# Parskatt/RoMa

Hardware: AMD Instinct MI355X
Metric: image-pairs/sec, roma_outdoor 560->864, batch=8 per GPU (higher is better)
Workload: dtype bf16; 1 GPU; roma_outdoor match() 560->864, symmetric, upsample_preds, 8 pairs/GPU/step, seeded synthetic weights + N(0,1) images; precision policy of the reference's bf16 timing script: bfloat16 DINOv2 + float16 autocast for VGG / decoder / refiners (ROMA_MIXED), f32 accumulate; precision_policy=mixed, global_batch=8, streams_per_gpu=2, parallelism=single GPU, outputs_finite=True

## Files before the change

### include/roma_hip.h

```cpp
#ifndef ROMA_HIP_H
#define ROMA_HIP_H
#include <stdint.h>
#ifdef __cplusplus
extern "C" {
#endif

typedef struct roma_model* roma_handle_t;

enum { ROMA_F32 = 0, ROMA_BF16 = 1, ROMA_F16 = 2,
       ROMA_MIXED = 3 };
int roma_h16_format(void);
enum { ROMA_ERR_ARG = -1, ROMA_ERR_HIP = -2, ROMA_ERR_STATE = -3 };

typedef struct {
  int coarse_h, coarse_w;
  int upsample_h, upsample_w;
  int symmetric;
  int upsample_preds;
  int attenuate_cert;
  int precision;
  int max_batch;
  int device;
} roma_config_t;

// ... 111 lines not shown
int roma_op_multinomial(const float* weights, long n, long k, unsigned long long seed, long long* out_indices, void* workspace,
                        long workspace_bytes, void* stream);
long roma_op_ransac_workspace(int B, int N);
int roma_op_ransac(int model, const float* kpts_a, const float* kpts_b, const int* counts, const unsigned long long* seeds, int B,
                   int N, float threshold, double confidence, int max_iters, int refine, double* out_model, unsigned char* out_mask,
                   unsigned char* out_ok, int* out_info, void* workspace, long workspace_bytes, void* stream);
long roma_op_magsac_workspace(int B, int N);
int roma_op_magsac(int model, const float* kpts_a, const float* kpts_b, const int* counts, const unsigned long long* seeds, int B,
                   int N, float threshold, double confidence, int max_iters, int lo_iters, double* out_model, unsigned char* out_mask,
                   unsigned char* out_ok, int* out_info, double* out_score, void* workspace, long workspace_bytes, void* stream);
long roma_op_essential_workspace(int B, int N);
int roma_op_essential(const float* kpts_a, const float* kpts_b, const int* counts, const unsigned long long* seeds,
                      const double* camera_matrix, int B, int N, float threshold, double prob, int max_iters, double* out_e,
                      unsigned char* out_mask, unsigned char* out_ok, int* out_info, void* workspace, long workspace_bytes,
                      void* stream);
long roma_op_essential_magsac_workspace(int B, int N);
int roma_op_essential_magsac(const float* kpts_a, const float* kpts_b, const int* counts, const unsigned long long* seeds,
                             const double* camera_matrix, int B, int N, float threshold, double prob, int max_iters, int lo_iters,
                             double* out_e, unsigned char* out_mask, unsigned char* out_ok, int* out_info, double* out_score,
                             void* workspace, long workspace_bytes, void* stream);
int roma_op_essential_minimal(const double* x0, const double* x1, int S, double* out_e, int* out_n, void* stream);
long roma_op_recover_pose_workspace(int B, int N);
int roma_op_recover_pose(const double* E, const float* kpts_a, const float* kpts_b, const unsigned char* mask, const int* counts,
                         const double* camera_matrix, int B, int N, double distance_thresh, int* out_n_good, double* out_r,
                         double* out_t, unsigned char* out_mask, void* workspace, long workspace_bytes, void* stream);
long roma_op_refine_pose_workspace(int B, int N);
int roma_op_refine_pose(const double* R, const double* t, const float* kpts_a, const float* kpts_b, const int* counts,
                        const unsigned char* valid, int B, int N, double thr, int max_steps, double* out_r, double* out_t,
                        unsigned char* out_mask, int* out_info, void* workspace, long workspace_bytes, void* stream);
long roma_op_refine_model_workspace(int B, int N);
int roma_op_refine_model(int model, const double* M, const float* kpts_a, const float* kpts_b, const int* counts,
                         const unsigned char* valid, int B, int N, double thr, int max_steps, double* out_m, unsigned char* out_mask,
                         int* out_info, double* out_cost, void* workspace, long workspace_bytes, void* stream);
int roma_op_nchw_to_nhwc(const float* in, float* out, int B, int C, int H, int W, void* stream);
int roma_op_tiny_pos_embed(const float* corr_volume, float* out, int B, int H1, int W1, int H0, int W0, int exact_softmax,
                           void* stream);
int roma_op_gray_instnorm(const float* in, float* out, int B, int H, int W, int C, float eps, void* stream);
int roma_op_conv2d_nhwc(const float* in, const float* w, const float* bias, const float* res, float* out, int B, int H, int W,
                        int Cin, int Cout, int K, int stride, int pad, int relu, void* stream);
int roma_op_avgpool_nhwc(const float* in, float* out, int B, int H, int W, int C, int k, void* stream);
int roma_op_add3(const float* a, const float* b, const float* c, float* out, long n, void* stream);
int roma_op_tiny_matcher_input(const float* f0, const float* f1, const float* warp, int warp_channels, float* d, int B, int H,
                               int W, int H1, int W1, int C, int Cp, void* stream);
int roma_op_tiny_update(const float* base, int base_channels, const float* delta, long ldd, float sx, float sy, float* out,
                        long npix, void* stream);
int roma_op_tiny_final(const float* matches, float* warp, float* certainty, int B, int H, int W, void* stream);
int roma_op_visualize_warp(const float* warp, const float* certainty, const float* im_a, const float* im_b, int H, int W,
                           int symmetric, int im_h, int im_w, float* out, void* stream);
int roma_op_fb_consistency(const float* flow_fwd, const float* flow_bwd, int B, int H, int W, float th_n, float* out,
                           void* stream);
int roma_op_maxpool2x2(const void* in, void* out, int B, int H, int W, int C, int dt, void* stream);
int roma_op_pool_proj(const void* in, void* pooled, void* pf, const void* pw, long ldw, const float* pb, int N, int ldf, int B, int H,
                      int W, int C, int dt, void* stream);
int roma_op_refiner_out(const void* d, long ldd, int dt, const float* w, const float* b, float* flow, float* cert, long M,
                        int Cp, float sx, float sy, void* stream);
int roma_op_conv3x3_c3(const float* img, const float* w, const float* bias, void* out, int B, int H, int W, int dt_out,
                       void* stream);
int roma_op_conv3x3_c3_bf16(const float* img, const void* w, const float* bias, void* out, int B, int H, int W, void* stream);

#ifdef __cplusplus
}
#endif
#endif
```

### roma_amd/_lib.py

```python
from __future__ import annotations

import ctypes as C
import os

_HERE = os.path.dirname(os.path.abspath(__file__))
_HERE = os.environ.get("ROMA_LIB_DIR", _HERE)
LIB_PATH = os.path.join(_HERE, "libroma_hip.so")
LIB_PATHS = {"bf16": LIB_PATH, "f16": os.path.join(_HERE, "libroma_hip_f16.so")}

ROMA_F32, ROMA_BF16, ROMA_F16, ROMA_MIXED = 0, 1, 2, 3
H16_CODE = {"bf16": ROMA_BF16, "f16": ROMA_F16}


class RomaConfig(C.Structure):
    _fields_ = [("coarse_h", C.c_int), ("coarse_w", C.c_int), ("upsample_h", C.c_int), ("upsample_w", C.c_int),
                ("symmetric", C.c_int), ("upsample_preds", C.c_int), ("attenuate_cert", C.c_int),
                ("precision", C.c_int), ("max_batch", C.c_int), ("device", C.c_int)]


class RomaForwardArgs(C.Structure):
    _fields_ = [("upsample", C.c_int), ("symmetric", C.c_int), ("scale_factor", C.c_double),
                ("seed_flow", C.c_void_p), ("seed_cert", C.c_void_p), ("seed_h", C.c_int), ("seed_w", C.c_int),
                ("flow", C.c_void_p * 5), ("cert", C.c_void_p * 5), ("feat", C.c_void_p * 5)]

# ... 27 lines not shown
    "roma_op_local_corr_window": (_i, [_vp, _vp, _vp, _vp, _i, _i, _i, _i, _i, _f, _l, _i, _i, _vp]),
    "roma_op_gemm": (_i, [_vp, _l, _vp, _l, _vp, _l, _i, _i, _i, _i, _l, _l, _l, _vp, _vp, _vp, _l, _i, _f, _i, _i, _vp]),
    "roma_op_conv3x3": (_i, [_vp, _vp, _vp, _vp, _i, _i, _i, _i, _i, _i, _i, _vp]),
    "roma_op_conv3x3_slab": (_i, [_vp, _vp, _vp, _vp, _i, _i, _i, _i, _i, _i, _i, _vp]),
    "roma_op_attention": (_i, [_vp, _vp, _vp, _vp, _i, _i, _i, _i, _i, _i, _i, _vp]),
    "roma_op_qkv_scatter_gemm": (_i, [_vp, _vp, _vp, _vp, _vp, _vp, _i, _i, _i, _i, _i, _i, _i, _i, _vp]),
    "roma_op_layernorm": (_i, [_vp, _vp, _vp, _vp, _l, _i, _f, _i, _vp]),
    "roma_op_layernorm_dt": (_i, [_vp, _i, _vp, _vp, _vp, _l, _i, _f, _i, _vp]),
    "roma_op_gemm_res_bf16": (_i, [_vp, _l, _vp, _l, _vp, _l, _i, _i, _i, _vp, _vp, _vp, _l, _vp]),
    "roma_op_cholesky_solve_t": (_i, [_vp, _vp, _vp, _vp, _vp, _i, _i, _i, _vp]),
    "roma_op_gp": (_i, [_vp, _vp, _vp, _vp, _vp, _i, _i, _i, _i, _vp]),
    "roma_op_cls_to_flow": (_i, [_vp, _l, _vp, _vp, _l, _vp]),
    "roma_op_resize_bilinear": (_i, [_vp, _vp, _i, _i, _i, _i, _i, _i, _vp]),
    "roma_op_refiner_input": (_i, [_vp, _l, _vp, _vp, _l, _vp, _vp, _i, _i, _i, _i, _i, _i, _i, _i, _f, _i, _vp]),
    "roma_op_dwconv5x5": (_i, [_vp, _vp, _vp, _vp, _i, _i, _i, _i, _i, _vp]),
    "roma_op_refiner_block": (_i, [_vp, _vp, _vp, _vp, _vp, _vp, _i, _i, _i, _i, _i, _vp]),
    "roma_op_refiner_block_final": (_i, [_vp, _vp, _vp, _vp, _vp, _vp, _i, _i, _i, _i, _i, _vp]),
    "roma_op_refiner_apply_delta": (_i, [_vp, _vp, _vp, _l, _f, _f, _vp]),
    "roma_op_kde": (_i, [_vp, _l, _i, _f, _i, _vp, _vp]),
    "roma_op_sample_warp_at": (_i, [_vp, _vp, _i, _i, _vp, _l, _vp, _vp, _vp]),
    "roma_op_mutual_nn": (_i, [_vp, _l, _vp, _l, _vp, _f, _f, _vp, _vp, _vp, _vp]),
    "roma_op_mutual_nn_count": (_i, [_vp, _l, _vp, _l, _vp, _f, _f, _vp, _vp, _vp, _vp]),
    "roma_op_mutual_nn_fill": (_i, [_vp, _l, _vp, _l, _vp, _f, _f, _vp, _vp, _vp, _vp, _vp]),
    "roma_op_fb_consistency": (_i, [_vp, _vp, _i, _i, _i, _f, _vp, _vp]),
    "roma_op_visualize_warp": (_i, [_vp, _vp, _vp, _vp, _i, _i, _i, _i, _i, _vp, _vp]),
    "roma_op_multinomial_workspace": (_l, [_l, _l]),
    "roma_op_multinomial": (_i, [_vp, _l, _l, C.c_ulonglong, _vp, _vp, _l, _vp]),
    "roma_op_ransac_workspace": (_l, [_i, _i]),
    "roma_op_ransac": (_i, [_i, _vp, _vp, _vp, _vp, _i, _i, _f, C.c_double, _i, _i, _vp, _vp, _vp, _vp, _vp, _l, _vp]),
    "roma_op_magsac_workspace": (_l, [_i, _i]),
    "roma_op_magsac": (_i, [_i, _vp, _vp, _vp, _vp, _i, _i, _f, C.c_double, _i, _i, _vp, _vp, _vp, _vp, _vp, _vp, _l, _vp]),
    "roma_op_essential_workspace": (_l, [_i, _i]),
    "roma_op_essential": (_i, [_vp, _vp, _vp, _vp, _vp, _i, _i, _f, C.c_double, _i, _vp, _vp, _vp, _vp, _vp, _l, _vp]),
    "roma_op_essential_magsac_workspace": (_l, [_i, _i]),
    "roma_op_essential_magsac": (_i, [_vp, _vp, _vp, _vp, _vp, _i, _i, _f, C.c_double, _i, _i, _vp, _vp, _vp, _vp, _vp, _vp, _l, _vp]),
    "roma_op_essential_minimal": (_i, [_vp, _vp, _i, _vp, _vp, _vp]),
    "roma_op_recover_pose_workspace": (_l, [_i, _i]),
    "roma_op_recover_pose": (_i, [_vp, _vp, _vp, _vp, _vp, _vp, _i, _i, C.c_double, _vp, _vp, _vp, _vp, _vp, _l, _vp]),
    "roma_op_refine_pose_workspace": (_l, [_i, _i]),
    "roma_op_refine_pose": (_i, [_vp, _vp, _vp, _vp, _vp, _vp, _i, _i, C.c_double, _i, _vp, _vp, _vp, _vp, _vp, _l, _vp]),
    "roma_op_refine_model_workspace": (_l, [_i, _i]),
    "roma_op_refine_model": (_i, [_i, _vp, _vp, _vp, _vp, _vp, _i, _i, C.c_double, _i, _vp, _vp, _vp, _vp, _vp, _l, _vp]),
    "roma_op_nchw_to_nhwc": (_i, [_vp, _vp, _i, _i, _i, _i, _vp]),
    "roma_op_tiny_pos_embed": (_i, [_vp, _vp, _i, _i, _i, _i, _i, _i, _vp]),
    "roma_op_gray_instnorm": (_i, [_vp, _vp, _i, _i, _i, _i, _f, _vp]),
    "roma_op_conv2d_nhwc": (_i, [_vp, _vp, _vp, _vp, _vp, _i, _i, _i, _i, _i, _i, _i, _i, _i, _vp]),
    "roma_op_avgpool_nhwc": (_i, [_vp, _vp, _i, _i, _i, _i, _i, _vp]),
    "roma_op_add3": (_i, [_vp, _vp, _vp, _vp, _l, _vp]),
    "roma_op_tiny_matcher_input": (_i, [_vp, _vp, _vp, _i, _vp, _i, _i, _i, _i, _i, _i, _i, _vp]),
    "roma_op_tiny_update": (_i, [_vp, _i, _vp, _l, _f, _f, _vp, _l, _vp]),
    "roma_op_tiny_final": (_i, [_vp, _vp, _vp, _i, _i, _i, _vp]),
    "roma_op_maxpool2x2": (_i, [_vp, _vp, _i, _i, _i, _i, _i, _vp]),
    "roma_op_pool_proj": (_i, [_vp, _vp, _vp, _vp, _l, _vp, _i, _i, _i, _i, _i, _i, _i, _vp]),
    "roma_op_conv3x3_c3": (_i, [_vp, _vp, _vp, _vp, _i, _i, _i, _i, _vp]),
    "roma_op_conv3x3_c3_bf16": (_i, [_vp, _vp, _vp, _vp, _i, _i, _i, _vp]),
    "roma_op_refiner_out": (_i, [_vp, _l, _i, _vp, _vp, _vp, _vp, _l, _i, _f, _f, _vp]),
}

_libs = {}


class RomaHipError(RuntimeError):
    pass


def load(fmt: str = "bf16"):
    if fmt in _libs:
        return _libs[fmt]
    path = LIB_PATHS[fmt]
    if not os.path.exists(path):
        raise ImportError(f"{path} not found - build it with `python -c 'import __graft_entry__ as g; g.build()'` "
                          "(roma_amd has no CPU fallback)")
    lib = C.CDLL(path)
    for name, (res, args) in SIGNATURES.items():
        fn = getattr(lib, name)
        fn.restype = res
        fn.argtypes = args
    if lib.roma_h16_format() != H16_CODE[fmt]:
        raise ImportError(f"{path} does not store {fmt} (roma_h16_format() = {lib.roma_h16_format()})")
    lib.h16 = fmt
    _libs[fmt] = lib
    return lib


def fmt_of(dtype) -> str:
    return "f16" if str(dtype) == "torch.float16" else "bf16"


def last_error(lib=None) -> str:
    return (lib or load()).roma_last_error().decode("utf-8", "replace")


def check(rc: int, exc=RomaHipError, lib=None):
    if rc != 0:
        raise exc(last_error(lib))
    return rc
```

### roma_amd/csrc/api.hip

```cpp
#include <algorithm>
#include <mutex>
#include <map>
#include <vector>
#include <dlfcn.h>
#include <string.h>

#include "../../include/roma_hip.h"
#include "attention.h"
#include "conv64.h"
#include "conv_patch.h"
#include "elementwise.h"
#include "gemm.h"
#include "local_corr.h"
#include "pool_proj.h"
#include "model.h"
#include "refiner_block.h"
#include "kde.h"
#include "keypoints.h"
#include "tiny.h"
#include "vit.h"
#include "sampling.h"
#include "essential.h"
#include "model_refine.h"
#include "pose_refine.h"
#include "geometry.h"

namespace roma {
static thread_local std::string g_err;
void set_error(const std::string& msg) { g_err = msg; }
}

namespace roma {
struct ProfRec { std::string name, unit; double work; hipEvent_t e0, e1; };
static bool g_prof_on = false;
static std::vector<ProfRec> g_prof;
bool prof_enabled() { return g_prof_on; }
void prof_begin(const char* kernel, double work, const char* unit, hipStream_t s) {
  ProfRec r;
  r.name = kernel; r.unit = unit; r.work = work;
  (void)hipEventCreate(&r.e0);
  (void)hipEventCreate(&r.e1);
  (void)hipEventRecord(r.e0, s);
  g_prof.push_back(r);
}
void prof_end(hipStream_t s) { (void)hipEventRecord(g_prof.back().e1, s); }
}

struct roma_model {
  roma::Model m;
};

namespace roma {
void* g_peer_lib = nullptr;
int g_mixed_handles = 0;
template <typename F> static F peer_sym(const char* name) {
  return g_peer_lib ? reinterpret_cast<F>(dlsym(g_peer_lib, name)) : nullptr;
}
}

using namespace roma;

static inline hipStream_t S(void* s) { return static_cast<hipStream_t>(s); }
// ... 133 lines not shown
                      long names_bytes) {
  if (!h || slot < 0 || slot >= Model::MAX_STREAMS_DECL) return ROMA_ERR_ARG;
  const long n = h->m.trace_n[slot];
  if (!sums_host) return n;
  if (max_entries < n || !h->m.trace_dev[slot]) {
    set_error("roma_debug_trace: destination too small or tracing was never enabled");
    return ROMA_ERR_ARG;
  }
  if (hipSetDevice(h->m.cfg.device) != hipSuccess || hipDeviceSynchronize() != hipSuccess) return ROMA_ERR_HIP;
  if (hipMemcpy(sums_host, h->m.trace_dev[slot], (size_t)n * sizeof(unsigned long long), hipMemcpyDeviceToHost) != hipSuccess)
    return ROMA_ERR_HIP;
  if (names_host && names_bytes > 0) {
    std::string all;
    for (long i = 0; i < n; ++i) all += h->m.trace_names[slot][(size_t)i] + "\n";
    const size_t c = std::min<size_t>(all.size(), (size_t)names_bytes - 1);
    memcpy(names_host, all.data(), c);
    names_host[c] = 0;
  }
  return n;
}

int roma_destroy(roma_handle_t h) {
  delete h;
  return 0;
}

int roma_tuning(const char* key, int value) {
  ROMA_REQUIRE(key, "roma_tuning: null key");
  if (g_mixed_handles > 0)
    if (auto f = peer_sym<int (*)(const char*, int)>("roma_tuning"))
      if (int rc = f(key, value)) {
        set_error(std::string("roma_tuning: the bfloat16 sibling library refused key ") + key);
        return rc;
      }
  const std::string k(key);
  if (k == "gemm8p") g_gemm_tuning[0] = value;
  else if (k == "gemm_dbg") g_gemm_tuning[1] = value;
  else if (k == "gemm8p_walk") g_gemm8p_walk = value;
  else if (k == "gemm8p_sched") g_gemm8p_sched = value;
  else if (k == "gemm8p_maxwg") g_gemm8p_maxwg = value;
  else if (k == "ws1x1") g_ws1x1_mode = value;
  else if (k == "lc_mode") g_lc_mode = value;
  else if (k == "lc_bin") g_lc_bin = value;
  else if (k == "conv64") g_conv64_mode = value;
  else if (k == "conv_patch") g_conv_patch = value;
  else if (k == "attn_xcd") g_attn_xcd_map = value;
  else if (k == "attn_exp2") g_attn_exp2 = value;
  else if (k == "rb24w") g_rb24_wave = value;
  else if (k == "rb144_1b") g_rb144_1b = value;
  else if (k == "rb_wide") g_rb_wide = value;
  else if (k == "dw_ring") g_dw_ring = value;
  else if (k == "gp_col") g_gp_col = value;
  else if (k == "pool_proj") g_pool_proj = value;
  else if (k == "gp_col_leader") g_gp_col_leader = value;
  else {
    set_error("roma_tuning: unknown key " + k);
    return ROMA_ERR_ARG;
  }
  return 0;
}

int roma_vit_forward(const roma_vit_args_t* a, void* stream) {
  ROMA_REQUIRE(a, "roma_vit_forward: null argument");
  ROMA_REQUIRE(a->act == ROMA_F32 || a->act == ROMA_H16_CODE, "roma_vit_forward: act must be ROMA_F32 or this library's 16-bit code");
  return vit_forward(*a, S(stream));
}

int roma_op_convert_from_bf16(const void* in_bf16, void* out_h16, long n, void* stream) {
  ROMA_REQUIRE(in_bf16 && out_h16, "roma_op_convert_from_bf16: null pointer");
  return convert_from_bf16_launch(in_bf16, out_h16, n, S(stream));
}

long roma_debug_gemm_trace(unsigned int* dst_host, long nbytes) {
  ROMA_REQUIRE(dst_host && nbytes > 0, "roma_debug_gemm_trace: null destination");
  if (hipDeviceSynchronize() != hipSuccess) return ROMA_ERR_HIP;
  const int rc = gemm8p_trace_read(dst_host, nbytes);
  return rc < 0 ? rc : std::min<long>(nbytes, (long)sizeof(unsigned) * 16 * 2 * 256 * 4);
}

int roma_profile_enable(int on) {
  if (g_mixed_handles > 0)
    if (auto f = peer_sym<int (*)(int)>("roma_profile_enable"))
      if (int rc = f(on)) return rc;
  for (auto& r : g_prof) { (void)hipEventDestroy(r.e0); (void)hipEventDestroy(r.e1); }
  g_prof.clear();
  g_prof_on = on != 0;
  return 0;
}

long roma_profile_report(char* buf, long nbytes) {
  if (hipDeviceSynchronize() != hipSuccess) return ROMA_ERR_HIP;
  struct Agg { long calls = 0; double ms = 0, work = 0; std::string unit; };
  std::map<std::string, Agg> agg;
  for (auto& r : g_prof) {
    float ms = 0.f;
    if (hipEventElapsedTime(&ms, r.e0, r.e1) != hipSuccess) continue;
    Agg& a = agg[r.name];
    a.calls++; a.ms += ms; a.work += r.work; a.unit = r.unit;
  }
  std::string js = "{";
  bool first = true;
  for (auto& kv : agg) {
    char tmp[512];
    snprintf(tmp, sizeof tmp, "%s\"%s\": {\"calls\": %ld, \"total_ms\": %.6f, \"work\": %.6e, \"unit\": \"%s\"}", first ? "" : ", ",
             kv.first.c_str(), kv.second.calls, kv.second.ms, kv.second.work, kv.second.unit.c_str());
    js += tmp;
// ... 262 lines not shown
                         int* out_info, double* out_cost, void* workspace, long workspace_bytes, void* stream) {
  return refine_model_launch(model, M, kpts_a, kpts_b, counts, valid, B, N, thr, max_steps, out_m, out_mask, out_info, out_cost,
                             workspace, (size_t)(workspace_bytes > 0 ? workspace_bytes : 0), S(stream));
}
int roma_op_nchw_to_nhwc(const float* in, float* out, int B, int C, int H, int W, void* stream) {
  return nchw_to_nhwc_launch(in, out, B, C, H, W, S(stream));
}
int roma_op_tiny_pos_embed(const float* corr_volume, float* out, int B, int H1, int W1, int H0, int W0, int exact_softmax,
                           void* stream) {
  return tiny_pos_embed_launch(corr_volume, out, B, H1, W1, H0, W0, exact_softmax, S(stream));
}
int roma_op_gray_instnorm(const float* in, float* out, int B, int H, int W, int C, float eps, void* stream) {
  return gray_instnorm_launch(in, out, B, H, W, C, eps, S(stream));
}
int roma_op_conv2d_nhwc(const float* in, const float* w, const float* bias, const float* res, float* out, int B, int H, int W,
                        int Cin, int Cout, int K, int stride, int pad, int relu, void* stream) {
  return conv2d_nhwc_launch(in, w, bias, res, out, B, H, W, Cin, Cout, K, stride, pad, relu, S(stream));
}
int roma_op_avgpool_nhwc(const float* in, float* out, int B, int H, int W, int C, int k, void* stream) {
  return avgpool_nhwc_launch(in, out, B, H, W, C, k, S(stream));
}
int roma_op_add3(const float* a, const float* b, const float* c, float* out, long n, void* stream) {
  return add3_launch(a, b, c, out, n, S(stream));
}
int roma_op_tiny_matcher_input(const float* f0, const float* f1, const float* warp, int warp_channels, float* d, int B, int H,
                               int W, int H1, int W1, int C, int Cp, void* stream) {
  return tiny_matcher_input_launch(f0, f1, warp, warp_channels, d, B, H, W, H1, W1, C, Cp, S(stream));
}
int roma_op_tiny_update(const float* base, int base_channels, const float* delta, long ldd, float sx, float sy, float* out,
                        long npix, void* stream) {
  return tiny_update_launch(base, base_channels, delta, ldd, sx, sy, out, npix, S(stream));
}
int roma_op_tiny_final(const float* matches, float* warp, float* certainty, int B, int H, int W, void* stream) {
  return tiny_final_launch(matches, warp, certainty, B, H, W, S(stream));
}
int roma_op_visualize_warp(const float* warp, const float* certainty, const float* im_a, const float* im_b, int H, int W,
                           int symmetric, int im_h, int im_w, float* out, void* stream) {
  return visualize_warp_launch(warp, certainty, im_a, im_b, H, W, symmetric, im_h, im_w, out, S(stream));
}
int roma_op_fb_consistency(const float* flow_fwd, const float* flow_bwd, int B, int H, int W, float th_n, float* out,
                           void* stream) {
  return fb_consistency_launch(flow_fwd, flow_bwd, B, H, W, th_n, out, S(stream));
}

int roma_op_maxpool2x2(const void* in, void* out, int B, int H, int W, int C, int dt, void* stream) {
  return maxpool2x2_launch(in, out, B, H, W, C, DT(dt), S(stream));
}

int roma_op_pool_proj(const void* in, void* pooled, void* pf, const void* pw, long ldw, const float* pb, int N, int ldf, int B, int H,
                      int W, int C, int dt, void* stream) {
  return pool_proj_launch(in, pooled, pf, pw, ldw, pb, N, ldf, B, H, W, C, DT(dt), S(stream));
}

int roma_op_refiner_out(const void* d, long ldd, int dt, const float* w, const float* b, float* flow, float* cert, long M,
                        int Cp, float sx, float sy, void* stream) {
  ROMA_REQUIRE(d && w && b && flow && cert && M > 0 && Cp > 0 && ldd >= Cp, "roma_op_refiner_out: bad arguments");
  return refiner_out_launch(d, ldd, DT(dt), w, b, flow, cert, M, Cp, sx, sy, S(stream));
}

int roma_op_conv3x3_c3_bf16(const float* img, const void* w, const float* bias, void* out, int B, int H, int W, void* stream) {
  return conv3x3_c3_bf16_launch(img, w, bias, out, B, H, W, S(stream));
}

int roma_op_conv3x3_c3(const float* img, const float* w, const float* bias, void* out, int B, int H, int W, int dt_out,
                       void* stream) {
  return conv3x3_c3_launch(img, w, bias, out, B, H, W, DT(dt_out), S(stream));
}

}
```

### roma_amd/csrc/model.hip

```cpp
#include "model.h"

#include <dlfcn.h>
#include <math.h>
#include <stdlib.h>
#include <string.h>

#include <algorithm>
#include <atomic>
#include <set>

#include "attention.h"
#include "conv64.h"
#include "pool_proj.h"
#include "elementwise.h"
#include "gemm.h"
#include "local_corr.h"
#include "refiner_block.h"
#include "vit.h"

namespace roma {

std::mutex g_peer_mutex;
extern void* g_peer_lib;
extern int g_mixed_handles;

static const int VGG_IDX[12] = {0, 3, 7, 10, 14, 17, 20, 23, 27, 30, 33, 36};
static const int VGG_CH[12] = {64, 64, 128, 128, 256, 256, 256, 256, 512, 512, 512, 512};
static const char* SCALES[5] = {"16", "8", "4", "2", "1"};
static const int SCALE_INT[5] = {16, 8, 4, 2, 1};
static const int PROJ_CIN[5] = {1024, 512, 256, 128, 64};
static const int PROJ_COUT[5] = {512, 512, 256, 64, 9};
static const int REF_EMB[5] = {128, 64, 32, 16, 6};
static const int REF_RAD[5] = {7, 3, 2, 0, 0};

Model::~Model() {
  for (int i = 0; i < MAX_STREAMS - 1; ++i) {
    if (side[i]) (void)hipStreamDestroy(side[i]);
    if (ev_join[i]) (void)hipEventDestroy(ev_join[i]);
  }
  if (ev_fork) (void)hipEventDestroy(ev_fork);
  for (void* p : owned) (void)hipFree(p);
  for (auto& kv : dbg) (void)hipFree(kv.second.first);
  for (auto& kv : inject) (void)hipFree(kv.second.first);
  if (peer_lib) {
    std::lock_guard<std::mutex> lk(g_peer_mutex);
    --g_mixed_handles;
  }
}


int Model::load_peer() {
  static void* lib = nullptr;
  static int (*fwd)(const roma_vit_args_t*, void*) = nullptr;
  std::lock_guard<std::mutex> lk(g_peer_mutex);
  if (!lib) {
    ROMA_REQUIRE(roma_h16_format() == ROMA_F16, "ROMA_MIXED is a mode of the binary16 build (libroma_hip_f16.so)");
    Dl_info info;
    ROMA_REQUIRE(dladdr(reinterpret_cast<void*>(&roma_vit_forward), &info) && info.dli_fname, "ROMA_MIXED: cannot locate this library");
    std::string path(info.dli_fname);
    const size_t slash = path.find_last_of('/');
    path = (slash == std::string::npos ? std::string("") : path.substr(0, slash + 1)) + "libroma_hip.so";
    void* l = dlopen(path.c_str(), RTLD_NOW | RTLD_LOCAL | RTLD_DEEPBIND);
    if (!l) {
      set_error("ROMA_MIXED: cannot load the bfloat16 library " + path + ": " + (dlerror() ? dlerror() : "?"));
      return ROMA_ERR_STATE;
// ... 823 lines not shown
    const size_t pass_mark = arena.mark();
    void* feat[5] = {nullptr};
    const int fh[4] = {H, H / 2, H / 4, H / 8}, fw_[4] = {W, W / 2, W / 4, W / 8};
    const int fc[4] = {64, 128, 256, 512};
    for (int l = 0; l < 4; ++l) feat[l] = AL((size_t)nimg * fh[l] * fw_[l] * fc[l], esz);
    static const bool pp_env = !(getenv("ROMA_POOL_PROJ") && atoi(getenv("ROMA_POOL_PROJ")) == 0);
    void* pf_pre[2] = {nullptr, nullptr};
    const int pp_si[2] = {4, 3};
    bool pp_on[2];
    for (int l = 0; l < 2; ++l) {
      const RefinerW& rr = ref[pp_si[l]];
      const int ldf_l = (int)round_up(rr.Cf, 8);
      pp_on[l] = (g_pool_proj >= 0 ? g_pool_proj != 0 : pp_env) && fh[l] >= 2 && fw_[l] >= 2 &&
                 pool_proj_supported(fc[l], rr.Cf, ldf_l, act_dt) && proj[pp_si[l]].b != nullptr;
      if (pp_on[l] || dry) pf_pre[l] = AL((size_t)nimg * fh[l] * fw_[l] * ldf_l, esz);
      if (!pp_on[l] && !dry) pf_pre[l] = nullptr;
    }
    {
      const size_t enc_mark = arena.mark();
      void* t0 = AL((size_t)nimg * H * W * 64, esz);
      void* t1 = AL((size_t)nimg * (H / 2) * (W / 2) * 64, esz);
      static const int c64_env = getenv("ROMA_CONV64") ? atoi(getenv("ROMA_CONV64")) : 7;
      void* col1 = AL((size_t)nimg * H * W * 32, esz);
      if (act_dt == DT_BF16 && ((g_conv64_mode >= 0 ? g_conv64_mode : c64_env) & 4) && (long)3 * H * W < (1l << 23)) {
        RUN(conv3x3_c3_bf16_launch(imA, vgg[0].w, vgg[0].b, t0, B, H, W, st));
        RUN(conv3x3_c3_bf16_launch(imB, vgg[0].w, vgg[0].b, off(t0, (long)B * H * W * 64), B, H, W, st));
      } else {
        RUN(im2col3x3_c3_launch(imA, col1, B, H, W, act_dt, st));
        RUN(im2col3x3_c3_launch(imB, off(col1, (long)B * H * W * 32), B, H, W, act_dt, st));
        GemmArgs g;
        g.A = col1; g.lda = 32; g.W = vgg[0].w; g.ldw = vgg[0].ldw; g.C = t0; g.ldc = 64;
        g.M = nimg * H * W; g.N = 64; g.K = 32; g.k_alg = 27; g.in_dt = act_dt; g.out_dt = act_dt; g.bias = vgg[0].b; g.act = ACT_RELU;
        RUN(gemm_launch(g, st));
      }
      auto conv = [&](int li, const void* in, void* out, int h, int w) -> int {
        GemmArgs g;
        g.A = in; g.W = vgg[li].w; g.ldw = vgg[li].ldw; g.C = out; g.ldc = vgg_cout[li];
        g.M = nimg * h * w; g.N = vgg_cout[li]; g.K = 9 * vgg_cin[li];
        g.in_dt = act_dt; g.out_dt = act_dt; g.bias = vgg[li].b; g.act = ACT_RELU;
        g.conv_h = h; g.conv_w = w; g.conv_c = vgg_cin[li]; g.conv_korder = vgg_korder[li];
        RUN(gemm_launch(g, st));
        return 0;
      };
      auto pool = [&](int l, const void* in, void* out) -> int {
        if (pp_on[l]) {
          const int si_ = pp_si[l];
          RUN(pool_proj_launch(in, out, pf_pre[l], proj[si_].w, proj[si_].ldw, proj[si_].b, ref[si_].Cf, (int)round_up(ref[si_].Cf, 8),
                               nimg, fh[l], fw_[l], fc[l], act_dt, st));
        } else {
          RUN(maxpool2x2_launch(in, out, nimg, fh[l], fw_[l], fc[l], act_dt, st));
        }
        return 0;
      };
      if (int rc = conv(1, t0, feat[0], H, W)) return rc;
      if (int rc = pool(0, feat[0], t1)) return rc;
      if (int rc = conv(2, t1, t0, H / 2, W / 2)) return rc;
      if (int rc = conv(3, t0, feat[1], H / 2, W / 2)) return rc;
      if (int rc = pool(1, feat[1], t1)) return rc;
      if (int rc = conv(4, t1, t0, H / 4, W / 4)) return rc;
      if (int rc = conv(5, t0, t1, H / 4, W / 4)) return rc;
      if (int rc = conv(6, t1, t0, H / 4, W / 4)) return rc;
      if (int rc = conv(7, t0, feat[2], H / 4, W / 4)) return rc;
      RUN(maxpool2x2_launch(feat[2], t1, nimg, H / 4, W / 4, 256, act_dt, st));
      if (int rc = conv(8, t1, t0, H / 8, W / 8)) return rc;
      if (int rc = conv(9, t0, t1, H / 8, W / 8)) return rc;
      if (int rc = conv(10, t1, t0, H / 8, W / 8)) return rc;
      if (int rc = conv(11, t0, feat[3], H / 8, W / 8)) return rc;
      arena.release(enc_mark);
    }
    for (int l = 0; l < 4; ++l)
      if (int rc = CK((up ? "p2_feat" : "p1_feat") + std::to_string(1 << l), feat[l], (size_t)nimg * fh[l] * fw_[l] * fc[l] * esz)) return rc;
    if (fw && !dry)
      for (int l = 0; l < 4; ++l)
        if (fw->feat[4 - l])
          ROMA_CHECK_HIP(hipMemcpyAsync(fw->feat[4 - l], feat[l], (size_t)nimg * fh[l] * fw_[l] * fc[l] * esz, hipMemcpyDeviceToDevice, st));
    if (debug && !dry && !up) {
      for (int l = 0; l < 4; ++l) {
        const std::string nm = "feat" + std::to_string(1 << l);
        if (int rc = dbg_save(nm.c_str(), feat[l], (size_t)nimg * fh[l] * fw_[l] * fc[l] * esz, st)) return rc;
      }
    }
    const long rows_d = (long)nimg * Nd, rows_t = (long)ndp * T;
    void *ln = nullptr, *ao = nullptr, *hid = nullptr;
    if (!up) {
      feat[4] = AL((size_t)nimg * T * 1024, esz);
      const long rmax = std::max(rows_d, rows_t);
      ln = AL((size_t)rmax * 1024, esz);
      ao = AL((size_t)rmax * 1024, esz);
      hid = AL((size_t)rmax * 4096, esz);
      const size_t dmark = arena.mark();
      void* col = AL((size_t)nimg * T * patch.ldw, esz);
      float* pt = (float*)AL((size_t)nimg * T * 1024, 4);
      float* x = (float*)AL((size_t)rows_d * 1024, 4);
      static const bool res_f32_env = getenv("ROMA_VIT_RES_F32") && atoi(getenv("ROMA_VIT_RES_F32")) != 0;
      void* xs = nullptr;
      if (act_dt == DT_BF16) xs = AL((size_t)rows_d * 1024, 2);
      void* feat_vit = feat[4];
      if (mixed) feat_vit = AL((size_t)nimg * T * 1024, 2);
      if (!dry) {
        roma_vit_block_t blk[24];
        for (int i = 0; i < 24; ++i) blk[i] = dino[i].pub();
        roma_vit_args_t va{};
        va.B = B; va.H = H; va.W = W;
        va.act = act_dt == DT_F32 ? ROMA_F32 : (mixed ? ROMA_BF16 : roma_h16_format());
        va.bf16_residual = act_dt == DT_BF16 && vit_bf16_residual && !res_f32_env;
        va.im_a = imA; va.im_b = imB;
        va.patch_w = patch.w; va.patch_b = patch.b; va.patch_ldw = patch.ldw;
        va.cls_tok = cls_tok; va.pos_emb = pos_emb;
// ... 267 lines not shown
```

Before: 107.0 image-pairs/s.

## Fuse first VGG 3x3 conv with maxpool and fine-scale projection

```diff
diff --git a/include/roma_hip.h b/include/roma_hip.h
--- a/include/roma_hip.h
+++ b/include/roma_hip.h
@@ -187,6 +187,8 @@
 int roma_op_maxpool2x2(const void* in, void* out, int B, int H, int W, int C, int dt, void* stream);
 int roma_op_pool_proj(const void* in, void* pooled, void* pf, const void* pw, long ldw, const float* pb, int N, int ldf, int B, int H,
                       int W, int C, int dt, void* stream);
+int roma_op_conv3x3_pool_proj(const void* in, const void* w, const float* bias, void* pooled, void* pf, const void* pw, long ldw,
+                              const float* pb, int N, int ldf, int B, int H, int W, int C, int dt, int sy, void* stream);
 int roma_op_refiner_out(const void* d, long ldd, int dt, const float* w, const float* b, float* flow, float* cert, long M,
                         int Cp, float sx, float sy, void* stream);
 int roma_op_conv3x3_c3(const float* img, const float* w, const float* bias, void* out, int B, int H, int W, int dt_out,
diff --git a/roma_amd/_lib.py b/roma_amd/_lib.py
--- a/roma_amd/_lib.py
+++ b/roma_amd/_lib.py
@@ -103,6 +103,7 @@
     "roma_op_tiny_final": (_i, [_vp, _vp, _vp, _i, _i, _i, _vp]),
     "roma_op_maxpool2x2": (_i, [_vp, _vp, _i, _i, _i, _i, _i, _vp]),
     "roma_op_pool_proj": (_i, [_vp, _vp, _vp, _vp, _l, _vp, _i, _i, _i, _i, _i, _i, _i, _vp]),
+    "roma_op_conv3x3_pool_proj": (_i, [_vp, _vp, _vp, _vp, _vp, _vp, _l, _vp, _i, _i, _i, _i, _i, _i, _i, _i, _vp]),
     "roma_op_conv3x3_c3": (_i, [_vp, _vp, _vp, _vp, _i, _i, _i, _i, _vp]),
     "roma_op_conv3x3_c3_bf16": (_i, [_vp, _vp, _vp, _vp, _i, _i, _i, _vp]),
     "roma_op_refiner_out": (_i, [_vp, _l, _i, _vp, _vp, _vp, _vp, _l, _i, _f, _f, _vp]),
diff --git a/roma_amd/csrc/api.hip b/roma_amd/csrc/api.hip
--- a/roma_amd/csrc/api.hip
+++ b/roma_amd/csrc/api.hip
@@ -8,6 +8,7 @@
 #include "../../include/roma_hip.h"
 #include "attention.h"
 #include "conv64.h"
+#include "conv_pool.h"
 #include "conv_patch.h"
 #include "elementwise.h"
 #include "gemm.h"
@@ -247,6 +248,7 @@
   else if (k == "dw_ring") g_dw_ring = value;
   else if (k == "gp_col") g_gp_col = value;
   else if (k == "pool_proj") g_pool_proj = value;
+  else if (k == "conv_pool") g_conv_pool = value;
   else if (k == "gp_col_leader") g_gp_col_leader = value;
   else {
     set_error("roma_tuning: unknown key " + k);
@@ -615,6 +617,11 @@
   return pool_proj_launch(in, pooled, pf, pw, ldw, pb, N, ldf, B, H, W, C, DT(dt), S(stream));
 }
 
+int roma_op_conv3x3_pool_proj(const void* in, const void* w, const float* bias, void* pooled, void* pf, const void* pw, long ldw,
+                              const float* pb, int N, int ldf, int B, int H, int W, int C, int dt, int sy, void* stream) {
+  return conv_pool_launch(in, w, bias, pooled, pf, pw, ldw, pb, N, ldf, B, H, W, C, DT(dt), sy, S(stream));
+}
+
 int roma_op_refiner_out(const void* d, long ldd, int dt, const float* w, const float* b, float* flow, float* cert, long M,
                         int Cp, float sx, float sy, void* stream) {
   ROMA_REQUIRE(d && w && b && flow && cert && M > 0 && Cp > 0 && ldd >= Cp, "roma_op_refiner_out: bad arguments");
diff --git a/roma_amd/csrc/conv_pool.h b/roma_amd/csrc/conv_pool.h
--- /dev/null
+++ b/roma_amd/csrc/conv_pool.h
@@ -0,0 +1,11 @@
+#pragma once
+#include "common.h"
+
+namespace roma {
+
+bool conv_pool_supported(int C, int N, int ldf, int dt, int H, int W);
+int conv_pool_launch(const void* in, const void* w, const float* bias, void* pooled, void* pf, const void* pw, long ldw,
+                     const float* pb, int N, int ldf, int nimg, int H, int W, int C, int dt, int sy_force, hipStream_t stream);
+extern int g_conv_pool;
+
+}
diff --git a/roma_amd/csrc/conv_pool.hip b/roma_amd/csrc/conv_pool.hip
--- /dev/null
+++ b/roma_amd/csrc/conv_pool.hip
@@ -0,0 +1,353 @@
+#include "conv_pool.h"
+
+#include <stdio.h>
+#include <stdlib.h>
+
+#include <algorithm>
+
+#include "gemm.h"
+#include "gemm_device.h"
+
+namespace roma {
+
+int g_conv_pool = -1;
+
+namespace {
+typedef unsigned u32x4 __attribute__((ext_vector_type(4)));
+typedef unsigned short u16x8 __attribute__((ext_vector_type(8)));
+
+__device__ __forceinline__ u32x4 pk_max_u16(u32x4 a, u32x4 b) {
+  return __builtin_bit_cast(u32x4, __builtin_elementwise_max(__builtin_bit_cast(u16x8, a), __builtin_bit_cast(u16x8, b)));
+}
+}
+
+constexpr int CP_TW = 128;
+constexpr int CP_NPIECE = ((CP_TW + 2) * 128 + 1023) / 1024;
+constexpr int CP_RSTRIDE = CP_NPIECE * 1024;
+constexpr int CP_BIAS = 4 * CP_RSTRIDE;
+constexpr int CP_PW = CP_BIAS + 512;
+constexpr int CP_POOL = CP_PW + 2048;
+constexpr int CP_LDS = CP_POOL + 8192;
+
+#define CP_WAIT_VM(N) asm volatile("s_waitcnt vmcnt(%0)" ::"n"(N) : "memory")
+
+__global__ __launch_bounds__(256, 2) void conv3x3_c64_pool_proj_kernel(const bf16_t* __restrict__ in, const bf16_t* __restrict__ w,
+                                                                       const float* __restrict__ bias, bf16_t* __restrict__ pooled,
+                                                                       bf16_t* __restrict__ pf, const bf16_t* __restrict__ pw, long ldw,
+                                                                       const float* __restrict__ pb, int N, int B, int H, int W,
+                                                                       int SY, int nxt, int nblocks) {
+  constexpr int TW = CP_TW, NPIECE = CP_NPIECE, RSTRIDE = CP_RSTRIDE;
+  constexpr int KW = (NPIECE + 3) / 4;
+  constexpr int LDF = 16;
+  extern __shared__ __attribute__((aligned(1024))) unsigned char ring[];
+
+  if ((int)blockIdx.x >= nblocks) return;
+  const int tid = threadIdx.x, lane = tid & 63;
+  const int wave = __builtin_amdgcn_readfirstlane(tid >> 6);
+  const int cg = wave & 1, pg = wave >> 1;
+  const int l31 = lane & 31, h = lane >> 5;
+  const unsigned ring0 = (unsigned)(size_t)((__attribute__((address_space(3))) unsigned char*)ring);
+
+  u32x4 wreg[36];
+  {
+    const bf16_t* wp = w + (long)(32 * cg + l31) * 576 + 8 * h;
+#pragma unroll
+    for (int ks = 0; ks < 36; ++ks) wreg[ks] = *reinterpret_cast<const u32x4*>(wp + 16 * ks);
+  }
+  {
+    float* bias_s = reinterpret_cast<float*>(ring + CP_BIAS);
+    if (tid < 64) bias_s[tid] = bias[tid];
+    if (tid >= 64 && tid < 64 + LDF) bias_s[tid] = tid - 64 < N ? pb[tid - 64] : 0.f;
+    if (tid >= 128) {
+      const int c = tid - 128, j = c & 15, hh = (c >> 4) & 1, ks = c >> 5;
+      u32x4 v = {0u, 0u, 0u, 0u};
+      if (j < N) v = *reinterpret_cast<const u32x4*>(pw + (long)j * ldw + 16 * ks + 8 * hh);
+      *reinterpret_cast<u32x4*>(ring + CP_PW + ((ks * 16 + j) * 2 + hh) * 16) = v;
+    }
+  }
+
+  unsigned rdo[3];
+#pragma unroll
+  for (int dx = 0; dx < 3; ++dx) {
+    const int p = 64 * pg + l31 + dx;
+    rdo[dx] = ring0 + (unsigned)(p * 128 + ((h ^ ((p >> 1) & 7)) << 4));
+  }
+
+  for (int lb = blockIdx.x; lb < nblocks; lb += gridDim.x) {
+  const int xt = lb % nxt;
+  const int r = lb / nxt;
+  const int yt = (H + SY - 1) / SY;
+  const int ys = (r % yt) * SY;
+  const int b = r / yt;
+  const int x0 = xt * TW;
+  const int sy = min(SY, H - ys);
+  if (lb != (int)blockIdx.x) __builtin_amdgcn_s_barrier();
+  asm volatile("" : "+v"(rdo[0]), "+v"(rdo[1]), "+v"(rdo[2]));
+
+  const bf16_t* inb = in + (long)b * H * W * 64;
+  const __amdgpu_buffer_rsrc_t rs_in = __builtin_amdgcn_make_buffer_rsrc(const_cast<bf16_t*>(inb), 0, (int)((long)H * W * 128), 0x00020000);
+  unsigned voff[KW];
+  bool okx[KW];
+  {
+    int gl = lane;
+    asm volatile("" : "+v"(gl));
+    const int dl_p = gl >> 3, dl_slot = gl & 7;
+    const u32x4 z4 = {0u, 0u, 0u, 0u};
+#pragma unroll
+    for (int j = 0; j < KW; ++j) {
+      const int q = wave + 4 * j;
+      const int p = q * 8 + dl_p;
+      const int x = x0 - 1 + p;
+      const int c = dl_slot ^ ((p >> 1) & 7);
+      okx[j] = q < NPIECE && p < TW + 2 && x >= 0 && x < W;
+      voff[j] = okx[j] ? (unsigned)(x * 128 + c * 16) : 0u;
+      if (q < NPIECE && !okx[j]) {
+#pragma unroll
+        for (int sl = 0; sl < 4; ++sl)
+          asm volatile("ds_write_b128 %0, %1 offset:%2" ::"v"(ring0 + sl * RSTRIDE + wave * 1024 + gl * 16), "v"(z4), "n"(j * 4096) : "memory");
+      }
+    }
+  }
+  asm volatile("s_waitcnt vmcnt(0) lgkmcnt(0)" ::: "memory");
+
+#define CP_ISSUE_ROW(YY, SLOT)                                                                                 \
+  {                                                                                                            \
+    const int yy_ = (YY);                                                                                      \
+    int ln_ = lane;                                                                                            \
+    asm volatile("" : "+v"(ln_));                                                                              \
+    const unsigned zb_ = ring0 + (SLOT) * RSTRIDE + wave * 1024 + ln_ * 16;       \
+    if (yy_ >= 0 && yy_ < H) {                                                                                 \
+      const int so_ = yy_ * W * 128;                                                                           \
+      _Pragma("unroll") for (int j = 0; j < KW; ++j) {                                                         \
+        const int q_ = wave + 4 * j;                                                                           \
+        if (q_ < NPIECE) {                                                                                     \
+          if (okx[j])                                                                                          \
+            __builtin_amdgcn_raw_ptr_buffer_load_lds(rs_in, (__attribute__((address_space(3))) void*)(ring + (SLOT) * RSTRIDE + q_ * 1024), \
+                                                     16, (int)voff[j], so_, 0, 0);                             \
+          else                                                                                                 \
+            asm volatile("ds_write_b128 %0, %1 offset:%2" ::"v"(zb_), "v"(u32x4{0u, 0u, 0u, 0u}), "n"(j * 4096) : "memory"); \
+        }                                                                                                      \
+      }                                                                                                        \
+    } else {                                     \
+      _Pragma("unroll") for (int j = 0; j < KW; ++j) {                                                         \
+        const int q_ = wave + 4 * j;                                                                           \
+        if (q_ < NPIECE)                                                                                       \
+          asm volatile("ds_write_b128 %0, %1 offset:%2" ::"v"(zb_), "v"(u32x4{0u, 0u, 0u, 0u}), "n"(j * 4096) : "memory"); \
+      }                                                                                                        \
+    }                                                                                                          \
+  }
+
+  u32x4 fa[2][4];
+#define CP_READ_G(SLOTOFF, DX, G)                                                                             \
+  {                                                                                                           \
+    const unsigned ad_ = (rdo[DX] + (SLOTOFF)) ^ (unsigned)((G) << 5);                                         \
+    asm volatile("ds_read_b128 %0, %1" : "=v"(fa[0][G]) : "v"(ad_));                                           \
+    asm volatile("ds_read_b128 %0, %1 offset:4096" : "=v"(fa[1][G]) : "v"(ad_));                              \
+  }
+#define CP_WAIT_G(G, N) asm volatile("s_waitcnt lgkmcnt(%2)" : "+v"(fa[0][G]), "+v"(fa[1][G]) : "n"(N) : "memory")
+
+  CP_ISSUE_ROW(ys - 1, 0)
+  CP_ISSUE_ROW(ys, 1)
+  CP_ISSUE_ROW(ys + 1, 2)
+
+  const int Ho = H >> 1, Wo = W >> 1;
+  for (int o = 0; o < sy; ++o) {
+    asm volatile("s_waitcnt vmcnt(0) lgkmcnt(0)" ::: "memory");
+    __builtin_amdgcn_s_barrier();
+    CP_ISSUE_ROW(ys + o + 2, (o + 3) & 3)
+    if (o == 0) {
+      CP_READ_G(0, 0, 0)
+      CP_READ_G(0, 0, 1)
+    }
+    CP_READ_G((o & 3) * RSTRIDE, 0, 2)
+    CP_READ_G((o & 3) * RSTRIDE, 0, 3)
+
+    f32x16 acc[2];
+#pragma unroll
+    for (int tm = 0; tm < 2; ++tm)
+#pragma unroll
+      for (int e = 0; e < 16; ++e) acc[tm][e] = 0.f;
+#pragma unroll
+    for (int t = 0; t < 9; ++t) {
+#pragma unroll
+      for (int g = 0; g < 4; ++g) {
+        if (t == 8 && g == 3) {
+          CP_WAIT_G(g, 4);
+        } else {
+          CP_WAIT_G(g, 6);
+        }
+#pragma unroll
+        for (int tm = 0; tm < 2; ++tm)
+          acc[tm] = mfma_h16_32x32x16(wreg[t * 4 + g],
+                                                            fa[tm][g], acc[tm]);
+        __builtin_amdgcn_sched_barrier(0);
+        if (t + 1 < 9) {
+          CP_READ_G(((o + (t + 1) / 3) & 3) * RSTRIDE, (t + 1) % 3, g)
+        } else if (g < 2) {
+          CP_READ_G(((o + 1) & 3) * RSTRIDE, 0, g)
+        }
+        __builtin_amdgcn_sched_barrier(0);
+      }
+    }
+
+    const int y = ys + o;
+    int el = lane;
+    asm volatile("" : "+v"(el));
+    const int e31 = el & 31, eh = el >> 5;
+    u32x4 st[2][2];
+#pragma unroll
+    for (int P = 0; P < 2; ++P) {
+      f32x4 bv0, bv1;
+      {
+        const unsigned ba = ring0 + CP_BIAS + (32 * cg + 16 * P + 4 * eh) * 4;
+        asm volatile("ds_read_b128 %0, %2\n\tds_read_b128 %1, %2 offset:32\n\ts_waitcnt lgkmcnt(0)"
+                     : "=&v"(bv0), "=&v"(bv1)
+                     : "v"(ba)
+                     : "memory");
+      }
+#pragma unroll
+      for (int tm = 0; tm < 2; ++tm) {
+        const unsigned a0 = pack_bf16x2(fmaxf(acc[tm][8 * P + 0] + bv0[0], 0.f), fmaxf(acc[tm][8 * P + 1] + bv0[1], 0.f));
+        const unsigned a1 = pack_bf16x2(fmaxf(acc[tm][8 * P + 2] + bv0[2], 0.f), fmaxf(acc[tm][8 * P + 3] + bv0[3], 0.f));
+        const unsigned b0 = pack_bf16x2(fmaxf(acc[tm][8 * P + 4] + bv1[0], 0.f), fmaxf(acc[tm][8 * P + 5] + bv1[1], 0.f));
+        const unsigned b1 = pack_bf16x2(fmaxf(acc[tm][8 * P + 6] + bv1[2], 0.f), fmaxf(acc[tm][8 * P + 7] + bv1[3], 0.f));
+        const auto s0 = __builtin_amdgcn_permlane32_swap(a0, b0, false, false);
+        const auto s1 = __builtin_amdgcn_permlane32_swap(a1, b1, false, false);
+        st[P][tm] = u32x4{s0[0], s1[0], s0[1], s1[1]};
+      }
+    }
+
+    u32x4 wf[2];
+    {
+      const unsigned wa = ring0 + CP_PW + (unsigned)(((2 * cg * 16 + (e31 & 15)) * 2 + eh) * 16);
+      asm volatile("ds_read_b128 %0, %2\n\tds_read_b128 %1, %2 offset:512\n\ts_waitcnt lgkmcnt(0)"
+                   : "=&v"(wf[0]), "=&v"(wf[1])
+                   : "v"(wa)
+                   : "memory");
+      if (e31 >= 16) wf[0] = wf[1] = u32x4{0u, 0u, 0u, 0u};
+    }
+    const unsigned xch = ring0 + (unsigned)((o & 3) * RSTRIDE + pg * 4096 + el * 16);
+    __builtin_amdgcn_s_barrier();
+    if (cg == 0) {
+#pragma unroll
+      for (int tm = 0; tm < 2; ++tm) {
+        f32x16 pa;
+#pragma unroll
+        for (int e = 0; e < 16; ++e) pa[e] = 0.f;
+        pa = mfma_h16_32x32x16(wf[0], st[0][tm], pa);
+        pa = mfma_h16_32x32x16(wf[1], st[1][tm], pa);
+        const f32x4 v0 = {pa[0], pa[1], pa[2], pa[3]}, v1 = {pa[4], pa[5], pa[6], pa[7]};
+        *reinterpret_cast<__attribute__((address_space(3))) f32x4*>(xch + tm * 2048) = v0;
+        *reinterpret_cast<__attribute__((address_space(3))) f32x4*>(xch + tm * 2048 + 1024) = v1;
+      }
+      asm volatile("s_waitcnt lgkmcnt(0)" ::: "memory");
+    }
+    __builtin_amdgcn_s_barrier();
+    if (cg == 1) {
+#pragma unroll
+      for (int tm = 0; tm < 2; ++tm) {
+        f32x4 v0, v1;
+        asm volatile("ds_read_b128 %0, %2\n\tds_read_b128 %1, %2 offset:1024\n\ts_waitcnt lgkmcnt(0)"
+                     : "=&v"(v0), "=&v"(v1)
+                     : "v"(xch + tm * 2048)
+                     : "memory");
+        f32x16 pa;
+#pragma unroll
+        for (int e = 0; e < 4; ++e) {
+          pa[e] = v0[e];
+          pa[4 + e] = v1[e];
+          pa[8 + e] = 0.f;
+          pa[12 + e] = 0.f;
+        }
+        pa = mfma_h16_32x32x16(wf[0], st[0][tm], pa);
+        pa = mfma_h16_32x32x16(wf[1], st[1][tm], pa);
+        f32x4 pbv0, pbv1;
+        asm volatile("ds_read_b128 %0, %2\n\tds_read_b128 %1, %2 offset:32\n\ts_waitcnt lgkmcnt(0)"
+                     : "=&v"(pbv0), "=&v"(pbv1)
+                     : "v"(ring0 + CP_BIAS + 256 + 16 * eh)
+                     : "memory");
+        const unsigned a0 = pack_bf16x2(pa[0] + pbv0[0], pa[1] + pbv0[1]), a1 = pack_bf16x2(pa[2] + pbv0[2], pa[3] + pbv0[3]);
+        const unsigned b0 = pack_bf16x2(pa[4] + pbv1[0], pa[5] + pbv1[1]), b1 = pack_bf16x2(pa[6] + pbv1[2], pa[7] + pbv1[3]);
+        const auto s0 = __builtin_amdgcn_permlane32_swap(a0, b0, false, false);
+        const auto s1 = __builtin_amdgcn_permlane32_swap(a1, b1, false, false);
+        const u32x4 pv = {s0[0], s1[0], s0[1], s1[1]};
+        const int x = x0 + 64 * pg + 32 * tm + e31;
+        if (x < W) *reinterpret_cast<u32x4*>(pf + (((long)b * H + y) * W + x) * LDF + 8 * eh) = pv;
+      }
+    }
+
+    {
+      const unsigned pa_ = ring0 + CP_POOL + (unsigned)(wave * 2048 + (el >> 1) * 16);
+      const bool even = !(e31 & 1);
+#pragma unroll
+      for (int P = 0; P < 2; ++P)
+#pragma unroll
+        for (int tm = 0; tm < 2; ++tm) {
+          const u32x4 m = st[P][tm];
+          u32x4 nbr;
+#pragma unroll
+          for (int i = 0; i < 4; ++i) nbr[i] = (unsigned)__shfl_down((int)m[i], 1);
+          const u32x4 hm = pk_max_u16(m, nbr);
+          const unsigned ad = pa_ + (P * 2 + tm) * 512;
+          if (!(o & 1)) {
+            if (even) asm volatile("ds_write_b128 %0, %1" ::"v"(ad), "v"(hm) : "memory");
+          } else {
+            u32x4 ev;
+            asm volatile("ds_read_b128 %0, %1\n\ts_waitcnt lgkmcnt(0)" : "=&v"(ev) : "v"(ad) : "memory");
+            const u32x4 mm = pk_max_u16(hm, ev);
+            const int x = x0 + 64 * pg + 32 * tm + e31;
+            if (even && x + 1 < W)
+              *reinterpret_cast<u32x4*>(pooled + (((long)b * Ho + (y >> 1)) * Wo + (x >> 1)) * 64 + 32 * cg + 16 * P + 8 * eh) = mm;
+          }
+        }
+    }
+  }
+  CP_WAIT_VM(0);
+  }
+#undef CP_WAIT_G
+#undef CP_READ_G
+#undef CP_ISSUE_ROW
+}
+
+bool conv_pool_supported(int C, int N, int ldf, int dt, int H, int W) {
+  return dt == DT_BF16 && C == 64 && N >= 1 && N <= 16 && ldf == 16 && H >= 2 && W >= 2 && (long)H * W * 128 < (1l << 31);
+}
+
+int conv_pool_launch(const void* in, const void* w, const float* bias, void* pooled, void* pf, const void* pw, long ldw,
+                     const float* pb, int N, int ldf, int nimg, int H, int W, int C, int dt, int sy_force, hipStream_t stream) {
+  ROMA_REQUIRE(conv_pool_supported(C, N, ldf, dt, H, W), "conv_pool: 16-bit maps with C = 64, N <= 16, ldf = 16 only");
+  ROMA_REQUIRE(in && w && bias && pooled && pf && pw && pb && nimg > 0 && ldw % 8 == 0 && ldw >= 64, "conv_pool: bad arguments");
+  const int slots = 512;
+  const int nxt = (W + CP_TW - 1) / CP_TW;
+  int SY = sy_force > 0 ? (sy_force + 1) & ~1 : 0;
+  if (SY <= 0) {
+    long best = -1;
+    for (int yt = 1; yt <= std::max(1, H / 12); ++yt) {
+      const int sy = ((H + yt - 1) / yt + 1) & ~1;
+      const long n = (long)nimg * nxt * ((H + sy - 1) / sy);
+      const long cost = ((n + slots - 1) / slots) * (sy + 3);
+      if (best < 0 || cost < best) {
+        best = cost;
+        SY = sy;
+      }
+    }
+  }
+  const long nb = (long)nimg * ((H + SY - 1) / SY) * nxt;
+  ROMA_REQUIRE(nb > 0 && nb < (1l << 30), "conv_pool: grid too large");
+  ProfScope ps("conv3x3_c64_pool_proj_kernel", 2.0 * (double)nimg * H * W * 64 * (576.0 + 16.0), "flop", stream);
+  static bool attr_set[64] = {false};
+  int dev = 0;
+  ROMA_CHECK_HIP(hipGetDevice(&dev));
+  if (dev < 0 || dev >= 64 || !attr_set[dev]) {
+    ROMA_CHECK_HIP(hipFuncSetAttribute(reinterpret_cast<const void*>(&conv3x3_c64_pool_proj_kernel), hipFuncAttributeMaxDynamicSharedMemorySize, CP_LDS));
+    if (dev >= 0 && dev < 64) attr_set[dev] = true;
+  }
+  const long gx = std::min<long>(nb, slots);
+  hipLaunchKernelGGL(conv3x3_c64_pool_proj_kernel, dim3((unsigned)gx), dim3(256), CP_LDS, stream, reinterpret_cast<const bf16_t*>(in),
+                     reinterpret_cast<const bf16_t*>(w), bias, reinterpret_cast<bf16_t*>(pooled), reinterpret_cast<bf16_t*>(pf),
+                     reinterpret_cast<const bf16_t*>(pw), ldw, pb, N, nimg, H, W, SY, nxt, (int)nb);
+  ROMA_LAUNCH_CHECK();
+  return 0;
+}
+
+}
diff --git a/roma_amd/csrc/model.hip b/roma_amd/csrc/model.hip
--- a/roma_amd/csrc/model.hip
+++ b/roma_amd/csrc/model.hip
@@ -11,6 +11,7 @@
 
 #include "attention.h"
 #include "conv64.h"
+#include "conv_pool.h"
 #include "pool_proj.h"
 #include "elementwise.h"
 #include "gemm.h"
@@ -940,8 +941,18 @@
         }
         return 0;
       };
-      if (int rc = conv(1, t0, feat[0], H, W)) return rc;
-      if (int rc = pool(0, feat[0], t1)) return rc;
+      static const bool cp_env = !(getenv("ROMA_CONV_POOL") && !(atoi(getenv("ROMA_CONV_POOL")) & 1));
+      const bool cp_on = (g_conv_pool >= 0 ? (g_conv_pool & 1) != 0 : cp_env) && pp_on[0] && !(fw && fw->feat[4]) && !debug && !tracing &&
+                         ((g_conv64_mode >= 0 ? g_conv64_mode : c64_env) & 1) && vgg_korder[1] == 0 && vgg[1].ldw == 576 &&
+                         conv_pool_supported(64, ref[pp_si[0]].Cf, (int)round_up(ref[pp_si[0]].Cf, 8), act_dt, H, W);
+      if (cp_on) {
+        const int si_ = pp_si[0];
+        RUN(conv_pool_launch(t0, vgg[1].w, vgg[1].b, t1, pf_pre[0], proj[si_].w, proj[si_].ldw, proj[si_].b, ref[si_].Cf,
+                             (int)round_up(ref[si_].Cf, 8), nimg, H, W, 64, act_dt, 0, st));
+      } else {
+        if (int rc = conv(1, t0, feat[0], H, W)) return rc;
+        if (int rc = pool(0, feat[0], t1)) return rc;
+      }
       if (int rc = conv(2, t1, t0, H / 2, W / 2)) return rc;
       if (int rc = conv(3, t0, feat[1], H / 2, W / 2)) return rc;
       if (int rc = pool(1, feat[1], t1)) return rc;
```

After: 107.4 image-pairs/s, median of 6. Within noise of the previous version (+0.4%).
